# friendlymatthew/heif

Hardware: AMD Instinct MI355X
Metric: Mpixels/s decoded (bit-exact) on 4032x3024 HEIC batch (higher is better)
Workload: dtype u8

## Files before the change

heif_amd/csrc/kernels/intra.hip:

```cpp
#include "kernels.hpp"
#include "intra_rec.hpp"
#include "xform.hpp"
#if defined(HG_HOST_EMU)
#include <cstdio>
#include <cstdlib>
#endif

namespace hg {

namespace {

constexpr int kMaxWaves = 16;
constexpr int kResidentIntraWaves = 4096;
constexpr size_t kIntraLdsBudget = 128 * 1024;

__constant__ int8_t c_angle[35] = {0, 0, 32, 26, 21, 17, 13, 9, 5, 2, 0, -2, -5, -9, -13, -17, -21, -26,
                                   -32, -26, -21, -17, -13, -9, -5, -2, 0, 2, 5, 9, 13, 17, 21, 26, 32};
__constant__ int16_t c_inv_angle[35] = {0, 0, 0, 0, 0, 0, 0, 0, 0, 0, 0, -4096, -1638, -910, -630, -482, -390, -315,
                                        -256, -315, -390, -482, -630, -910, -1638, -4096, 0, 0, 0, 0, 0, 0, 0, 0, 0};

struct alignas(16) IntraScratch {
    int16_t left[66];
    int16_t top[66];
    int16_t fl[66];
// ... 373 lines not shown
            const int p0 = *ang_ref(main_, side, inv, a + idx + 1), p1 = *ang_ref(main_, side, inv, a + idx + 2);
            pv = ((32 - fact) * p0 + fact * p1 + 16) >> 5;
            if (cidx == 0 && n < 32) {
                if (mode == 26) {
                    const int v = min(max(tp[1] + ((lf[1 + y] - lf[0]) >> 1), 0), maxv);
                    pv = x == 0 ? v : pv;
                }
                if (mode == 10) {
                    const int v = min(max(lf[1] + ((tp[1 + x] - tp[0]) >> 1), 0), maxv);
                    pv = y == 0 ? v : pv;
                }
            }
        }
        const int li = ((y0 + y) << w.lsx) + x0 + x;
        if (pcm) pv = 0;
        if (cbf) pv += (n <= 8 && o == lane) ? r0 : rt[y * w.rp + x];
        pv = min(max(pv, 0), maxv);
        w.cur[li] = (Pel)pv;
    };
#if defined(HG_IABL_PRED)
    if (lane == 1000) predict_sample(0);
    if (false)
#elif !defined(HG_HOST_EMU)
    if (n <= 8) {
        if (lane < n * n) predict_sample(lane);
    } else
#endif
    {
        for (int o = lane; o < n * n; o += kWave) predict_sample(o);
    }
    wave_sync();
}

#if !defined(HG_HOST_EMU)
template <typename Pel>
__device__ __attribute__((always_inline)) inline void predict_pair(IntraScratch *L, uint32_t wa, uint32_t wb,
                                                                   const TbWin<Pel> &wc, uint32_t dwin, uint32_t dres,
                                                                   int bd, int lane) {
    static_assert(kWave == 64, "predict_pair splits a 64-lane wave into two halves");
    const int log2n = tba_log2(wa), n = 1 << log2n, mode = tba_mode(wa);
    const int x0 = tba_lx(wa), y0 = tba_ly(wa);
    const int zc = tbb_zc(wb);
    const int h = lane >> 5, sl = lane & 31;
    TbWin<Pel> w = wc;
    const uint32_t dw = h ? dwin : 0u;
    w.cur = wc.cur + dw;
    w.left = wc.left + dw;
    w.above = wc.above + dw;
    const int16_t *rt = wc.rt + (h ? dres : 0u);
    const bool cbf = (wa & (h ? TBA_CBF2 : TBA_CBF)) != 0;
    const bool pcm = (wa & (h ? TBA_PCM2 : TBA_PCM)) != 0;
    const int csl = w.csl;
    const int ns = 4 * n + 1, nch = n == 8 ? 2 : 1;
    int r0 = 0, r1 = 0;
    if (cbf && sl < n * n) r0 = rt[(sl >> log2n) * w.rp + (sl & (n - 1))];
    if (cbf && sl + 32 < n * n) r1 = rt[((sl + 32) >> log2n) * w.rp + ((sl + 32) & (n - 1))];
    int16_t *left = L->left + 33 * h, *top = L->top + 33 * h;
    int val0 = 0, val1 = 0;
    uint32_t hm0 = 0, hm1 = 0;
#pragma unroll
    for (int k = 0; k < 2; ++k) {
        if (k >= nch) break;
        const int s = sl + 32 * k;
        const int xn = s <= 2 * n ? x0 - 1 : x0 + s - 2 * n - 1;
        const int yn = s < 2 * n ? y0 + 2 * n - 1 - s : y0 - 1;
        const bool av = s < ns && xn >= w.minx && yn >= w.miny && xn < w.vw && yn < w.vh &&
                        nb_avail(zc, xn * 2, yn * 2, csl);
        const Pel *srcp = w.at(xn, yn);
        const int vk = av ? (int)*srcp : 0;
        const uint32_t hk = (uint32_t)(__ballot(av) >> (32 * h));
        if (k == 0) {
            val0 = vk;
            hm0 = hk;
        } else {
            val1 = vk;
            hm1 = hk;
        }
    }
    const bool any = (hm0 | hm1) != 0;
#pragma unroll
    for (int k = 0; k < 2; ++k) {
        if (k >= nch) break;
        const int s = sl + 32 * k;
        const uint32_t hmk = k ? hm1 : hm0;
        int sc = k, src = sl;
        if (any && !((hmk >> sl) & 1u)) {
            const uint32_t below = hmk & ((1u << sl) - 1u);
            if (below) {
                src = 31 - __builtin_clz(below);
            } else if (k == 1 && hm0) {
                sc = 0;
                src = 31 - __builtin_clz(hm0);
            } else {
                sc = hm0 ? 0 : 1;
                src = __builtin_ctz(sc ? hm1 : hm0);
            }
        }
        const int v0 = __shfl(val0, 32 * h + src, 64);
        const int v1 = nch > 1 ? __shfl(val1, 32 * h + src, 64) : 0;
        const int v = !any ? (1 << (bd - 1)) : (sc == 0 ? v0 : v1);
        int16_t *dp = s < 2 * n ? left + (2 * n - s) : top + (s - 2 * n);
        if (s < ns) *dp = (int16_t)v;
        if (s == 2 * n) left[0] = (int16_t)v;
    }
    wave_sync();
    const int16_t *lf = left, *tp = top;
    const int maxv = (1 << bd) - 1;
    int dc = 0;
    const int ang = tbb_ang(wb), inv = tbb_inv(wb);
    const int16_t *main_ = mode >= 18 ? tp : lf, *side = mode >= 18 ? lf : tp;
    if (mode == 1) {
        const int sum = group_sum(sl < 2 * n ? (sl < n ? tp[1 + sl] : lf[1 + sl - n]) : 0, 2 * n);
        const int s0 = __builtin_amdgcn_readlane(sum, 0), s1 = __builtin_amdgcn_readlane(sum, 32);
        dc = ((h ? s1 : s0) + n) >> (log2n + 1);
    }
    for (int it = 0; it < nch; ++it) {
        const int o = sl + 32 * it;
        if (o < n * n) {
            const int x = o & (n - 1), y = o >> log2n;
            int pv;
            if (mode == 0) {
                pv = ((n - 1 - x) * lf[1 + y] + (x + 1) * tp[1 + n] + (n - 1 - y) * tp[1 + x] + (y + 1) * lf[1 + n] +
                      n) >> (log2n + 1);
            } else if (mode == 1) {
                pv = dc;
            } else {
                const int a = mode >= 18 ? x : y, b = mode >= 18 ? y : x;
                const int idx = ((b + 1) * ang) >> 5, fact = ((b + 1) * ang) & 31;
                const int p0 = *ang_ref(main_, side, inv, a + idx + 1), p1 = *ang_ref(main_, side, inv, a + idx + 2);
                pv = ((32 - fact) * p0 + fact * p1 + 16) >> 5;
            }
            if (pcm) pv = 0;
            if (cbf) pv += it ? r1 : r0;
            pv = min(max(pv, 0), maxv);
            w.cur[((y0 + y) << w.lsx) + x0 + x] = (Pel)pv;
        }
    }
    wave_sync();
}
#endif

}

#ifndef HG_INTRA_WPE
#define HG_INTRA_WPE 5
#endif
#if HG_INTRA_WPE > 0
#define HG_INTRA_ATTR __attribute__((amdgpu_waves_per_eu(HG_INTRA_WPE)))
#else
#define HG_INTRA_ATTR
#endif
constexpr size_t kXfTablesBytes = sizeof(XfTab);
constexpr size_t kXfDBytes = 32 * kXfDStride32 * sizeof(int16_t), kXfGBytes = 32 * 32 * sizeof(int16_t);
constexpr size_t kXfWaveBytes = kXfDBytes + kXfGBytes + 16;
static_assert(kXfTablesBytes % 16 == 0 && kXfWaveBytes % 16 == 0, "transform scratch alignment");
constexpr int kIntraPlanes = 0, kIntraStream = 1;

#if defined(HG_HOST_EMU)
struct LaneWord {
    uint32_t v[64];
    uint32_t at(int l) const { return v[l]; }
};
struct WalkStats {
    std::atomic<uint64_t> records{0}, ok{0}, pairs{0}, ctus{0}, blocks{0};
    std::atomic<uint64_t> pair_splits{0};
    std::atomic<uint64_t> ctu_lane0{0};
    std::atomic<uint64_t> blocks_no_ctu{0};
    std::atomic<uint64_t> rows_lt64{0}, rows_gt128{0};
    std::atomic<uint64_t> second_rows{0};
    std::atomic<uint64_t> tb32_strong{0}, luma4{0}, pcm{0};
};
static WalkStats g_walk;
static bool walk_stats_on() {
    static const bool on = [] {
        const char *e = std::getenv("HEIFGPU_INTRA_STATS");
        return e && std::atoi(e) != 0;
    }();
    return on;
}
#else
struct LaneWord {
    uint32_t v = 0;
    __device__ __forceinline__ uint32_t at(int l) const { return (uint32_t)__builtin_amdgcn_readlane((int)v, l); }
};
#endif
constexpr uint32_t kGaveUp = ~0u;
constexpr uint64_t kRedoPatience = 200000000ull;

template <typename Pel, int CF, int Mode>
__device__ __attribute__((always_inline)) inline void intra_body(const BatchArgs &a, unsigned char *smem) {
    constexpr bool Poll = Mode == kIntraStream;
    constexpr bool XfInline = Poll;
    const int nw = (int)HG_UNI(blockDim.x >> 6);
    const int pic = a.pic0 + blockIdx.x;
    const int wave = (int)HG_UNI(threadIdx.x >> 6), lane = threadIdx.x & 63;
    const PicDesc pd = a.pics[pic];
    if (pd.flags & PD_ASSEMBLY) return;
    if (Poll && a.stream_redo && hg_load_agent(a.xntu + a.total_rows + pic) != 0) return;
    const SeqParams sp = a.seqs[pd.seq];
    const int W = sp.width, H = sp.height, log2ctb = sp.log2_ctb;
    const int wctb = (W + (1 << log2ctb) - 1) >> log2ctb, hctb = (H + (1 << log2ctb) - 1) >> log2ctb;
    constexpr int chroma = CF;
    const int cw = chroma ? W >> chroma_sx(chroma) : 0, ch = chroma ? H >> chroma_sy(chroma) : 0;
    const int ncomp = chroma ? 3 : 1;
    const bool strong = (sp.flags & SP_STRONG_INTRA) != 0;
    const WinLayout lay = win_layout(log2ctb, chroma, (int)sizeof(Pel));
    uint32_t *progress = reinterpret_cast<uint32_t *>(smem);
    Frame<Pel, CF> F;
    F.blk = smem + 64 + (size_t)wave * lay.bytes;
    F.recon = reinterpret_cast<Pel *>(a.recon + pd.recon_off);
    F.resid = a.resid + pd.resid_off;
    F.init(log2ctb, W, H, cw, ch);
    XfScratch X{};
    if constexpr (XfInline) {
        unsigned char *tab = smem + 64 + (size_t)nw * lay.bytes;
        unsigned char *xw = tab + kXfTablesBytes + (size_t)wave * kXfWaveBytes;
        X = XfScratch{reinterpret_cast<int16_t *>(xw), reinterpret_cast<int16_t *>(xw + kXfDBytes),
                      reinterpret_cast<int32_t *>(xw + kXfDBytes + kXfGBytes), reinterpret_cast<const XfTab *>(tab)};
        xf_tables(reinterpret_cast<XfTab *>(tab), lane);
    }
    IntraScratch *S = reinterpret_cast<IntraScratch *>(F.blk);
    progress[wave] = 0;
    __syncthreads();
    const uint32_t stride = (uint32_t)wctb + 1;
    const bool split = a.intra_split != 0 && ncomp == 3;
    const int cls = split ? (wave & 1) : 0, rw = split ? wave >> 1 : wave, nrw = split ? nw >> 1 : nw;
    const int k0 = split && cls ? 1 : 0, k1 = split && !cls ? 1 : ncomp;
    const int prev_wave = split ? ((rw + nrw - 1) % nrw) * 2 + cls : (wave + nw - 1) % nw;
    const bool wpp = (sp.flags & SP_WPP) != 0;
    bool gave_up = false;
    const TbGeom G{log2ctb, chroma, W, H, cw, ch};
    const WinOffs wo = win_offs(F);
    constexpr int SX = chroma_sx(CF), SY = chroma_sy(CF);
    const uint32_t dwin = F.b1 / (uint32_t)sizeof(Pel);
    const uint32_t dres = (uint32_t)cw * (uint32_t)ch;
#if defined(HG_HOST_EMU)
    const bool stats = walk_stats_on() && cls == 0 && !(Poll && a.stream_redo);
    const bool stats_c = walk_stats_on() && k0 <= 1 && k1 > 1;
#endif
    for (int r = rw; r < hctb; r += nrw) {
        uint32_t ntu = Poll ? 0u : a.row_counts[2 * (pd.row_off + r)];
        bool row_done = !Poll;
        const TuRec *tus = a.tus + pd.tu_off + (uint64_t)r * pd.tu_cap_row;
        const CoefSrc<Poll> coefs{a.coefs + pd.coef_off + (uint64_t)r * pd.coef_cap_row};
        int cur = -1;
        auto finish_ctu = [&]() {
            _Pragma("nounroll") for (int k = 0; k < 3; ++k) {
                if (k >= ncomp) break;
                if (k < k0 || k >= k1) continue;
                const Win<Pel> w = F.win(k, cur, r);
                Pel *const plane = F.plane(k);
                const int PW = F.pw(k), PH = F.ph(k);
                const int vw = min(w.csx, PW - w.cx0), vh = min(w.csy, PH - w.cy0);
                if (vw == w.csx && !(PW & 3) && !(reinterpret_cast<uintptr_t>(plane) & (4 * sizeof(Pel) - 1))) {
                    const int lq = __builtin_ctz((unsigned)w.csx) - 2;
                    for (int o = lane; o < (vh << lq); o += kWave) {
                        const int x = (o & ((1 << lq) - 1)) << 2, y = o >> lq;
                        *reinterpret_cast<Quad<Pel> *>(plane + (size_t)(w.cy0 + y) * PW + w.cx0 + x) =
                            *reinterpret_cast<const Quad<Pel> *>(w.cur + y * w.csx + x);
                    }
                } else {
                    for (int o = lane; o < vw * vh; o += kWave) {
                        const int x = o % vw, y = o / vw;
                        plane[(size_t)(w.cy0 + y) * PW + w.cx0 + x] = w.cur[y * w.csx + x];
                    }
                }
                for (int y = lane; y < w.csy; y += kWave) w.left[y] = w.cur[y * w.csx + w.csx - 1];
            }
            wave_sync();
            HG_FENCE_REL();
            hg_atomic_store(&progress[wave], (uint32_t)r * stride + (uint32_t)cur + 1u);
        };
        auto start_ctu = [&](int c) -> bool {
            if (r > 0) {
                const uint32_t need = (uint32_t)(r - 1) * stride + (uint32_t)min(c + 2, wctb);
                for (uint32_t spin = 0;; ++spin) {
                    const uint32_t v = (uint32_t)HG_UNI(hg_atomic_load(&progress[prev_wave]));
                    if (Poll && v == kGaveUp) return false;
                    if (v >= need) break;
                    if (spin > (1u << 24)) {
                        if (lane == 0) atomicOr(&a.status[pic], ST_SUBSTREAM_END);
                        break;
                    }
                    HG_SLEEP();
                }
                HG_FENCE_ACQ();
            }
            _Pragma("nounroll") for (int k = 0; k < 3; ++k) {
                if (k >= ncomp) break;
                if (k < k0 || k >= k1) continue;
                const Win<Pel> w = F.win(k, c, r);
                const Pel *const plane = F.plane(k);
                const int PW = F.pw(k);
                const int yg = w.cy0 - 1;
                for (int i = lane; i <= 2 * w.csx; i += kWave) {
                    const int xg = w.cx0 - 1 + i;
                    w.above[i] = (yg >= 0 && xg >= 0 && xg < PW) ? plane[(size_t)yg * PW + xg] : (Pel)0;
                }
            }
            wave_sync();
            return true;
        };
#if defined(HG_HOST_EMU)
        if (stats) {
            g_walk.rows_lt64 += ntu < 64 && !Poll;
            g_walk.rows_gt128 += ntu > 128 && !Poll;
            g_walk.second_rows += r != rw;
        }
#endif
        bool stop = false;
        for (uint32_t t = 0; !stop;) {
            if constexpr (Poll) {
                if (t >= ntu && !row_done) {
                    const uint32_t *pw = a.xprog + pd.row_off + (wpp ? r : 0);
                    const uint32_t *nw_ = a.xntu + pd.row_off + r;
                    const uint32_t fin = (uint32_t)(r + 1) * (uint32_t)wctb;
                    const uint64_t patience = (uint64_t)a.stream_patience_us * 100u;
                    uint32_t seen_n = ~0u, seen_p = ~0u;
                    uint64_t t_last = 0;
                    for (;;) {
                        if (!a.stream_redo && !patience) {
                            gave_up = true;
                            break;
                        }
                        const uint32_t n_ = (uint32_t)HG_UNI(hg_load_agent(nw_));
                        if (n_ > t) {
                            ntu = n_;
                            break;
                        }
                        const uint32_t pv = (uint32_t)HG_UNI(hg_load_agent(pw));
                        if (pv >= fin) {
                            ntu = (uint32_t)HG_UNI(hg_load_agent(nw_));
                            row_done = true;
                            break;
                        }
                        const uint64_t now = hg_clock_10ns();
                        if (n_ != seen_n || pv != seen_p) {
                            seen_n = n_;
                            seen_p = pv;
                            t_last = now;
                        } else if (now - t_last > (a.stream_redo ? kRedoPatience : patience)) {
                            if (!a.stream_redo) {
                                gave_up = true;
                            } else {
                                if (lane == 0) atomicOr(&a.status[pic], ST_SUBSTREAM_END);
                                row_done = true;
                            }
                            break;
                        }
                        HG_STREAM_SLEEP();
                    }
                    if (gave_up) break;
                    HG_ACQ_AGENT();
                }
            }
            if (t >= ntu) break;
            const uint32_t base = t & ~63u;
            LaneWord wa, wb, wc, wctu;
#if !defined(HG_HOST_EMU)
            uint4 tblk = make_uint4(0, 0, 0, 0);
#endif
            auto form = [&](int l, uint32_t &A, uint32_t &B, uint32_t &C, uint32_t &ctu) {
                A = B = C = ctu = 0;
                const uint32_t i = base + (uint32_t)l;
                if (i < t || i >= ntu) return;
                TuRec q;
#if defined(HG_HOST_EMU)
                q = tus[i];
#else
                if constexpr (Poll) {
                    const uint64_t *p = reinterpret_cast<const uint64_t *>(tus + i);
// ... 338 lines not shown
```

heif_amd/csrc/kernels/transform.hip:

```cpp
#include "xform.hpp"

namespace hg {

namespace {

#ifndef HG_XF_WAVES
#define HG_XF_WAVES 4
#endif
constexpr int kWaves = HG_XF_WAVES;

#define wave_sync() HG_WAVE_SYNC()

}

#if !defined(HG_XF_WPE)
#define HG_XF_WPE 7
#endif
__global__ void __launch_bounds__(kWaves * 64) __attribute__((amdgpu_waves_per_eu(HG_XF_WPE))) k_transform(BatchArgs a) {
    HG_BLOCK_SHARED __attribute__((aligned(16))) int16_t dtile[kWaves][32 * kXfDStride32];
    HG_BLOCK_SHARED __attribute__((aligned(16))) int16_t gtile[kWaves][32 * 32];
    HG_BLOCK_SHARED int32_t extent[kWaves][2];
    HG_BLOCK_SHARED XfTab s_tab;
#if defined(HG_HOST_EMU)
    xf_tables(&s_tab, 0, 1);
#else
    xf_tables(&s_tab, (int)threadIdx.x, (int)blockDim.x);
#endif
    const int16_t *s_mt = s_tab.mt;
    __syncthreads();
    const int pic = a.pic0 + blockIdx.y, row = blockIdx.x;
    const PicDesc pd = a.pics[pic];
    if (pd.flags & PD_ASSEMBLY) return;
    const SeqParams sp = a.seqs[pd.seq];
    const int hctb = (sp.height + (1 << sp.log2_ctb) - 1) >> sp.log2_ctb;
    if (row >= hctb) return;
    const int wave = (int)HG_UNI(threadIdx.x >> 6), lane = threadIdx.x & 63;
    const uint32_t ntu = a.row_counts[2 * (pd.row_off + row)];
    const TuRec *tus = a.tus + pd.tu_off + (uint64_t)row * pd.tu_cap_row;
    const CoefSrc<false> coefs{a.coefs + pd.coef_off + (uint64_t)row * pd.coef_cap_row};
    const int W = sp.width, H = sp.height;
    const int cw = HG_UNI(sp.chroma_format ? W >> chroma_sx(sp.chroma_format) : 0);
    const int ch = HG_UNI(sp.chroma_format ? H >> chroma_sy(sp.chroma_format) : 0);
    int16_t HG_GAS *const res0 = (int16_t HG_GAS *)(a.resid + pd.resid_off);
    int16_t HG_GAS *res_plane[3] = {res0, res0 + (size_t)W * H, res0 + (size_t)W * H + (size_t)cw * ch};
    const int pitch[3] = {W, cw, cw};
    const bool scaling = (sp.flags & SP_SCALING_LIST) != 0;
    int16_t *d = dtile[wave];
    int16_t *g = gtile[wave];

    {
        const uint32_t mine = ntu > (uint32_t)wave ? (ntu - (uint32_t)wave + kWaves - 1) / kWaves : 0;
        auto want4 = [&](const TuRec &tu) -> bool {
            const int cidx = tu.flags & TU_CIDX_MASK;
            return (tu.flags & TU_CBF) && tu.log2 == 2 && cidx <= 2 && tu.x + 4 <= pitch[cidx] &&
                   tu.y + 4 <= (cidx ? ch : H);
        };
        auto round4 = [&](auto &&grp) {
            for (int vl = lane; vl < 64; vl += kWave) d[vl] = 0;
            wave_sync();
            for (int vl = lane; vl < 64; vl += kWave) {
                TuRec tu;
                const int l16 = vl & 15;
                if (!grp(vl, tu)) continue;
                const int cidx = tu.flags & TU_CIDX_MASK;
                const int bd = cidx ? sp.bit_depth_c : sp.bit_depth_y;
                int pos, dv;
                if (tu.flags & TU_PCM) {
                    if (l16 >= (int)tu.ncoef) continue;
                    const Coef c = coefs.word(tu.coef + (uint32_t)l16);
                    pos = (int)(c & 15u);
                    dv = (int)(int16_t)(c >> 16);
                } else {
                    if (tu.ncoef < 4) continue;
                    const SbRec r = load_rec(coefs, tu.coef);
                    if (!((r.sig() >> l16) & 1u)) continue;
                    const int above = l16 < 15 ? __builtin_popcountll(r.esc() >> (4 * l16 + 4)) : 0;
                    dv = r.level(l16, above, coefs);
                    pos = r.pos(l16, 2);
                }
                if (!(tu.flags & TU_BYPASS)) {
                    const int qp = tu.qp, bd_shift = bd - 3;
                    const int ls = c_level_scale[qp % 6] << (qp / 6);
                    const int m =
                        scaling ? a.sf[sp.sf_off + sf_size_offset(0) + (uint32_t)cidx * 16u + (uint32_t)pos] : 16;
                    dv = clip16(((int64_t)dv * m * ls + ((int64_t)1 << (bd_shift - 1))) >> bd_shift);
                }
                d[(vl & 48) + ((pos & 3) << 2) + (pos >> 2)] = (int16_t)dv;
            }
            wave_sync();
            for (int vl = lane; vl < 64; vl += kWave) {
                TuRec tu;
                if (!grp(vl, tu) || (tu.flags & (TU_BYPASS | TU_TSKIP))) continue;
                const int y = (vl & 15) >> 2, x = vl & 3;
                const uint32_t *pa = reinterpret_cast<const uint32_t *>(mt_of(s_mt, 2, (tu.flags & TU_DST) != 0) + y * 4);
                const uint32_t *pb = reinterpret_cast<const uint32_t *>(d + (vl & 48) + x * 4);
                const int s = dot2_i16(pa[1], pb[1], dot2_i16(pa[0], pb[0], 0));
                g[vl] = (int16_t)min(max((s + 64) >> 7, -32768), 32767);
            }
            wave_sync();
            for (int vl = lane; vl < 64; vl += kWave) {
                TuRec tu;
                if (!grp(vl, tu)) continue;
                const int cidx = tu.flags & TU_CIDX_MASK;
                const int bd2 = 20 - (cidx ? sp.bit_depth_c : sp.bit_depth_y);
                const int y = (vl & 15) >> 2, x = vl & 3;
                const int16_t *dq = d + (vl & 48), *gq = g + (vl & 48);
                int r;
                if (tu.flags & TU_BYPASS) {
                    r = dq[x * 4 + y];
                } else if (tu.flags & TU_TSKIP) {
                    r = (dq[x * 4 + y] * (1 << 7) + (1 << (bd2 - 1))) >> bd2;
                } else {
                    const uint32_t *pa = reinterpret_cast<const uint32_t *>(mt_of(s_mt, 2, (tu.flags & TU_DST) != 0) + x * 4);
                    const uint32_t *pb = reinterpret_cast<const uint32_t *>(gq + y * 4);
                    const int s = dot2_i16(pa[1], pb[1], dot2_i16(pa[0], pb[0], 0));
                    r = (s + (1 << (bd2 - 1))) >> bd2;
                }
                res_plane[cidx][(size_t)(tu.y + y) * pitch[cidx] + tu.x + x] = (int16_t)clip16(r);
            }
            wave_sync();
        };
#if defined(HG_HOST_EMU)
        for (uint32_t j = 0; j < mine; j += 4) {
            round4([&](int vl, TuRec &tu) -> bool {
                const uint32_t jq = j + (uint32_t)(vl >> 4);
                if (jq >= mine) return false;
                tu = tus[(uint32_t)wave + kWaves * jq];
                return want4(tu);
            });
        }
#else
        static_assert(kWave == 64, "one record per lane");
        for (uint32_t c0 = 0; c0 < mine; c0 += 64) {
            const uint32_t jl = c0 + (uint32_t)lane;
            uint4 rec = make_uint4(0, 0, 0, 0);
            if (jl < mine) rec = *reinterpret_cast<const uint4 *>(tus + (uint32_t)wave + kWaves * jl);
            TuRec rl;
            __builtin_memcpy(&rl, &rec, sizeof(rl));
            uint64_t todo = __ballot(jl < mine && want4(rl));
            while (todo) {
                int src = -1;
                for (int q = 0; q < 4 && todo; ++q) {
                    const int jq = __builtin_ctzll(todo);
                    todo &= todo - 1;
                    if (q == (lane >> 4)) src = jq;
                }
                const int sl = src < 0 ? 0 : src;
                const uint4 r = make_uint4((uint32_t)__shfl((int)rec.x, sl, 64), (uint32_t)__shfl((int)rec.y, sl, 64),
                                           (uint32_t)__shfl((int)rec.z, sl, 64), (uint32_t)__shfl((int)rec.w, sl, 64));
                TuRec tu_c;
                __builtin_memcpy(&tu_c, &r, sizeof(tu_c));
                const bool ok_c = src >= 0;
                round4([&](int, TuRec &tu) -> bool {
                    tu = tu_c;
                    return ok_c;
                });
            }
        }
#endif
    }

    auto pass_b = [&](const TuRec &tu) {
        const int cidx = tu.flags & TU_CIDX_MASK;
        transform_tb(tu, coefs, sp, a.sf, XfScratch{d, g, extent[wave], &s_tab},
                     res_plane[cidx] + (size_t)tu.y * pitch[cidx] + tu.x, pitch[cidx], lane);
    };
    auto wanted = [&](const TuRec &tu) {
        const int cidx = tu.flags & TU_CIDX_MASK, n = 1 << tu.log2;
        return (tu.flags & TU_CBF) && tu.log2 != 2 && tu.log2 <= 5 && cidx <= 2 && tu.x + n <= pitch[cidx] &&
               tu.y + n <= (cidx ? ch : H);
    };
#if defined(HG_HOST_EMU)
    for (uint32_t t = wave; t < ntu; t += kWaves)
        if (wanted(tus[t])) pass_b(tus[t]);
#else
    for (uint32_t t0 = wave; t0 < ntu; t0 += 64u * kWaves) {
        const uint32_t t = t0 + (uint32_t)lane * kWaves;
        uint4 rec = make_uint4(0, 0, 0, 0);
        if (t < ntu) rec = *reinterpret_cast<const uint4 *>(tus + t);
        TuRec mine;
        __builtin_memcpy(&mine, &rec, sizeof(mine));
        uint64_t todo = __ballot(t < ntu && wanted(mine));
        while (todo) {
            const int j = __builtin_ctzll(todo);
            todo &= todo - 1;
            const uint4 r = make_uint4((uint32_t)__builtin_amdgcn_readlane((int)rec.x, j),
                                       (uint32_t)__builtin_amdgcn_readlane((int)rec.y, j),
                                       (uint32_t)__builtin_amdgcn_readlane((int)rec.z, j),
                                       (uint32_t)__builtin_amdgcn_readlane((int)rec.w, j));
            TuRec tu;
            __builtin_memcpy(&tu, &r, sizeof(tu));
            pass_b(tu);
        }
    }
#endif
}

__global__ void __launch_bounds__(kWaves * 64) k_paint_flags(BatchArgs a) {
    const int pic = a.pic0 + blockIdx.y, row = blockIdx.x;
    const PicDesc pd = a.pics[pic];
    if (pd.flags & PD_ASSEMBLY) return;
    const SeqParams sp = a.seqs[pd.seq];
    const int hctb = (sp.height + (1 << sp.log2_ctb) - 1) >> sp.log2_ctb;
    if (row >= hctb) return;
    const int w4 = (sp.width + 3) >> 2, h4 = (sp.height + 3) >> 2;
    uint8_t *flg = a.maps + pd.map_off + (size_t)w4 * h4;
    const uint32_t ntu = min(a.row_counts[2 * (pd.row_off + row)], pd.tu_cap_row);
    const TuRec *tus = a.tus + pd.tu_off + (uint64_t)row * pd.tu_cap_row;
    const int wave = (int)(threadIdx.x >> 6), lane = threadIdx.x & 63;
    for (uint32_t t0 = 64u * wave; t0 < ntu; t0 += 64u * kWaves) {
        for (int vl = lane; vl < 64; vl += kWave) {
            const uint32_t t = t0 + (uint32_t)vl;
            if (t >= ntu) continue;
            const TuRec tu = tus[t];
            if ((tu.flags & (TU_CIDX_MASK | TU_PCM)) || tu.log2 < 2 || tu.log2 > 5) continue;
            const int nb = 1 << (tu.log2 - 2), gx0 = tu.x >> 2, gy0 = tu.y >> 2;
            if (gx0 >= w4 || gy0 >= h4) continue;
            const int wx = gx0 + nb <= w4 ? nb : w4 - gx0, hy = gy0 + nb <= h4 ? nb : h4 - gy0;
            const uint8_t nf = (tu.flags & TU_BYPASS) ? MF_NOFILT : 0;
            for (int y = 0; y < hy; ++y) {
                uint8_t *r = flg + (size_t)(gy0 + y) * w4 + gx0;
                const uint8_t h = (uint8_t)((y == 0 ? MF_EDGE_H : 0) | nf);
                const uint64_t v = (0x0101010101010101ull * h) | (uint64_t)MF_EDGE_V;
                if (wx == 8) {
                    __builtin_memcpy(r, &v, 8);
                } else if (wx == 4) {
                    __builtin_memcpy(r, &v, 4);
                } else {
                    for (int x = 0; x < wx; ++x) r[x] = (uint8_t)(v >> (8 * x));
                }
            }
        }
    }
    uint8_t *qmap = a.maps + pd.map_off;
    const int wctb = (sp.width + (1 << sp.log2_ctb) - 1) >> sp.log2_ctb;
    const uint32_t cap = cu_cap_row(wctb, sp.log2_ctb);
    const uint32_t ncu = min(a.cu_counts[pd.row_off + row], cap);
    const uint32_t *cus = a.cus + cu_list_off(pd.sao_off, a.max_log2ctb) + (uint64_t)row * cap;
    for (uint32_t t0 = 64u * wave; t0 < ncu; t0 += 64u * kWaves) {
        for (int vl = lane; vl < 64; vl += kWave) {
            const uint32_t t = t0 + (uint32_t)vl;
            if (t >= ncu) continue;
            const uint32_t w = cus[t];
            const int log2 = (int)((w >> 20) & 15u);
            if (log2 < 3 || log2 > 6) continue;
            const int nb = 1 << (log2 - 2), gx0 = (int)(w & 0xffffu) << 1;
            const int gy0 = (row << (sp.log2_ctb - 2)) + ((int)((w >> 16) & 15u) << 1);
            if (gx0 >= w4 || gy0 >= h4) continue;
            const int wx = gx0 + nb <= w4 ? nb : w4 - gx0, hy = gy0 + nb <= h4 ? nb : h4 - gy0;
            const uint64_t v = 0x0101010101010101ull * (uint64_t)(w >> 24);
            for (int y = 0; y < hy; ++y) {
                uint8_t *r = qmap + (size_t)(gy0 + y) * w4 + gx0;
                int x = 0;
                for (; x + 8 <= wx; x += 8) __builtin_memcpy(r + x, &v, 8);
                if (x + 4 <= wx) {
                    __builtin_memcpy(r + x, &v, 4);
                    x += 4;
                }
                for (; x < wx; ++x) r[x] = (uint8_t)v;
            }
        }
    }
}

#if defined(HG_HOST_EMU)
void emu_transform(const BatchArgs &a) {
    emu_launch(k_transform, a.max_rows, a.n_pics, kWaves, a);
    if (a.flags_from_recs) emu_launch(k_paint_flags, a.max_rows, a.n_pics, kWaves, a);
}
#else
hipError_t launch_transform(const BatchArgs &a, hipStream_t s) {
    hipLaunchKernelGGL(k_transform, dim3(a.max_rows, a.n_pics), dim3(kWaves * 64), 0, s, a);
    if (a.flags_from_recs) hipLaunchKernelGGL(k_paint_flags, dim3(a.max_rows, a.n_pics), dim3(kWaves * 64), 0, s, a);
    return hipGetLastError();
}
#endif

}
```

heif_amd/csrc/kernels/xform.hpp:

```cpp
#pragma once
#include "kernels.hpp"
#include "tables.hpp"

namespace hg {
namespace {

struct TransMatrix {
    int8_t m[32][32];
};
constexpr TransMatrix make_matrix() {
    TransMatrix t{};
    constexpr int odd[16] = {90, 90, 88, 85, 82, 78, 73, 67, 61, 54, 46, 38, 31, 22, 13, 4};
    constexpr int e2[8] = {90, 87, 80, 70, 57, 43, 25, 9};
    constexpr int e4[4] = {89, 75, 50, 18};
    int cv[33] = {};
    cv[0] = 64;
    cv[8] = 83;
    cv[16] = 64;
    cv[24] = 36;
    cv[32] = 0;
    for (int i = 0; i < 16; ++i) cv[2 * i + 1] = odd[i];
    for (int i = 0; i < 8; ++i) cv[2 * (2 * i + 1)] = e2[i];
    for (int i = 0; i < 4; ++i) cv[4 * (2 * i + 1)] = e4[i];
    for (int k = 0; k < 32; ++k)
        for (int n = 0; n < 32; ++n) {
            int j = ((2 * n + 1) * k) % 128;
            int v = j <= 32 ? cv[j] : j <= 64 ? -cv[64 - j] : j <= 96 ? -cv[j - 64] : cv[128 - j];
            t.m[k][n] = (int8_t)v;
        }
    return t;
}
__constant__ TransMatrix c_tm = make_matrix();
__constant__ int8_t c_dst[4][4] = {{29, 55, 74, 84}, {74, 74, 0, -74}, {84, -29, -74, 55}, {55, -84, 74, -29}};
__constant__ int16_t c_level_scale[6] = {40, 45, 51, 57, 64, 72};

#define xf_sync() HG_WAVE_SYNC()

__device__ __forceinline__ int clip16(int64_t v) { return v < -32768 ? -32768 : (v > 32767 ? 32767 : (int)v); }

template <bool Coherent>
struct CoefSrc {
    const Coef *p;
    __device__ __forceinline__ uint32_t word(uint32_t i) const {
#if !defined(HG_HOST_EMU)
        if constexpr (Coherent) return __hip_atomic_load(p + i, __ATOMIC_RELAXED, __HIP_MEMORY_SCOPE_AGENT);
#endif
        return p[i];
    }
};

struct SbRec {
    uint32_t w0, w1, w2, w3;
    __device__ __forceinline__ uint32_t sig() const { return w0 & 0xffffu; }
    __device__ __forceinline__ uint64_t nib() const { return (uint64_t)w1 | ((uint64_t)w2 << 32); }
    __device__ __forceinline__ uint64_t esc() const {
        const uint64_t x = nib();
        return x & (x >> 1) & (x >> 2) & (x >> 3) & 0x1111111111111111ull;
    }
    __device__ __forceinline__ uint32_t esc0() const { return w3 >> 9; }
    __device__ __forceinline__ int pos(int nn, int log2n) const {
        const uint32_t sc = (w3 >> 6) & 3u;
        const uint64_t sw = sc == 0 ? kScan4Pos[0] : (sc == 1 ? kScan4Pos[1] : kScan4Pos[2]);
        const uint32_t pp = (uint32_t)(sw >> (4 * nn)) & 15u;
        const int x = (int)((w3 & 7u) << 2) + (int)(pp & 3u), y = (int)(((w3 >> 3) & 7u) << 2) + (int)(pp >> 2);
        return (y << log2n) + x;
    }
    template <class Src>
    __device__ __forceinline__ int sum_abs(const Src &row) const {
        const uint64_t x = nib();
        const uint64_t t = (x & 0x0f0f0f0f0f0f0f0full) + ((x >> 4) & 0x0f0f0f0f0f0f0f0full);
        int s = __builtin_popcount(sig()) + (int)((t * 0x0101010101010101ull) >> 56);
        const int ne = __builtin_popcountll(esc());
        for (int k = 0; k < ne; ++k) s += (int)row.word(esc0() - (uint32_t)k) - 16;
        return s;
    }
    template <class Src>
    __device__ __forceinline__ int level(int nn, int esc_above, const Src &row) const {
        const int a = (int)((nib() >> (4 * nn)) & 15u);
        const int abs_v = a < 15 ? a + 1 : (int)row.word(esc0() - (uint32_t)esc_above);
        const uint32_t s = sig();
        bool neg;
        if (((w3 >> 8) & 1u) && nn == __builtin_ctz(s)) {
            neg = (sum_abs(row) & 1) != 0;
        } else {
            const int rank = __builtin_popcount(s >> (nn + 1));
            neg = ((w0 << rank) >> 31) != 0;
        }
        const int v = neg ? -abs_v : abs_v;
        return v < -32768 ? -32768 : (v > 32767 ? 32767 : v);
    }
};
template <bool Coherent>
__device__ __forceinline__ SbRec load_rec(const CoefSrc<Coherent> &src, uint32_t i) {
#if defined(HG_HOST_EMU)
    const Coef *p = src.p + i;
    return SbRec{p[0], p[1], p[2], p[3]};
#else
    if constexpr (Coherent) {
        const uint64_t *q = reinterpret_cast<const uint64_t *>(src.p + i);
        const uint64_t lo = __hip_atomic_load(q, __ATOMIC_RELAXED, __HIP_MEMORY_SCOPE_AGENT);
        const uint64_t hi = __hip_atomic_load(q + 1, __ATOMIC_RELAXED, __HIP_MEMORY_SCOPE_AGENT);
        return SbRec{(uint32_t)lo, (uint32_t)(lo >> 32), (uint32_t)hi, (uint32_t)(hi >> 32)};
    }
    const uint4 v = *reinterpret_cast<const uint4 *>(src.p + i);
    return SbRec{v.x, v.y, v.z, v.w};
#endif
}


constexpr int kXfDStride32 = 32 + 2;
constexpr int kMt4Dct = 8 * 10 + 16 * 18 + 32 * 34, kMt4Dst = kMt4Dct + 16;
constexpr int kMtElems = kMt4Dst + 16;
__device__ __forceinline__ int mt_off(int log2n) { return log2n == 3 ? 0 : (log2n == 4 ? 8 * 10 : 8 * 10 + 16 * 18); }

struct alignas(16) XfTab {
    int16_t mt[kMtElems];
};
static_assert(sizeof(XfTab) % 16 == 0 && (sizeof(int16_t) * kMtElems) % 16 == 0, "XfTab layout");

struct XfScratch {
    int16_t *d, *g;
    int32_t *extent;
    const XfTab *tab;
};

constexpr XfTab make_xf_tab() {
    XfTab t{};
    const TransMatrix m = make_matrix();
    constexpr int dst4[4][4] = {{29, 55, 74, 84}, {74, 74, 0, -74}, {84, -29, -74, 55}, {55, -84, 74, -29}};
    for (int i = 0; i < kMtElems; ++i) {
        if (i >= kMt4Dct) {
            const int k = i & 3, y = (i >> 2) & 3;
            t.mt[i] = (int16_t)(i >= kMt4Dst ? dst4[k][y] : m.m[k * 8][y]);
            continue;
        }
        const int l2 = i < 80 ? 3 : (i < 80 + 288 ? 4 : 5), n = 1 << l2, sn = n + 2;
        const int k = i - (l2 == 3 ? 0 : (l2 == 4 ? 80 : 80 + 288));
        const int y = k / sn, j = k % sn;
        t.mt[i] = (int16_t)(j < n ? m.m[j << (5 - l2)][y] : 0);
    }
    return t;
}
__constant__ XfTab c_xf = make_xf_tab();

__device__ __forceinline__ void xf_tables(XfTab *dst, int tid, int nth = kWave) {
    for (int i = tid; i < (int)(sizeof(XfTab) / 4); i += nth)
        reinterpret_cast<uint32_t *>(dst)[i] = reinterpret_cast<const uint32_t *>(&c_xf)[i];
}

#if !defined(HG_HOST_EMU) && !defined(HG_XF_NO_MFMA)
typedef int xf_v4i __attribute__((ext_vector_type(4)));
typedef int xf_v16i __attribute__((ext_vector_type(16)));
__device__ __forceinline__ int xf_hi(uint32_t w0, uint32_t w1) {
    return (int)__builtin_amdgcn_perm(w1, w0, 0x07050301u);
}
__device__ __forceinline__ int xf_lo(uint32_t w0, uint32_t w1) {
    return (int)(__builtin_amdgcn_perm(w1, w0, 0x06040200u) ^ 0x80808080u);
}
__device__ __forceinline__ int xf_hi4(int g0, int g1, int g2, int g3) {
    return (int)(__builtin_amdgcn_perm((uint32_t)g1, (uint32_t)g0, 0x0c0c0501u) |
                 (__builtin_amdgcn_perm((uint32_t)g3, (uint32_t)g2, 0x0c0c0501u) << 16));
}
__device__ __forceinline__ int xf_lo4(int g0, int g1, int g2, int g3) {
    return (int)((__builtin_amdgcn_perm((uint32_t)g1, (uint32_t)g0, 0x0c0c0400u) |
                  (__builtin_amdgcn_perm((uint32_t)g3, (uint32_t)g2, 0x0c0c0400u) << 16)) ^ 0x80808080u);
}
__device__ __forceinline__ int xf_b8(uint32_t w0, uint32_t w1) {
    return (int)__builtin_amdgcn_perm(w1, w0, 0x06040200u);
}
template <class DstPtr>
__device__ __forceinline__ void transform_mfma(const int16_t *dT, int sn, int log2n, const int16_t *mt, DstPtr dst,
                                               int pitch, int bd2, int lane) {
    const int n = 1 << log2n, r = lane & 31, h = lane >> 5;
    const bool live = r < n, live1 = live && 16 * h < n;
    const uint32_t *pm = reinterpret_cast<const uint32_t *>(mt + (live ? r : 0) * sn);
    const uint32_t *pm1 = pm + (live1 ? 8 * h : 0);
    const xf_v4i b1 = {live1 ? xf_b8(pm1[0], pm1[1]) : 0, live1 ? xf_b8(pm1[2], pm1[3]) : 0,
                       live1 ? xf_b8(pm1[4], pm1[5]) : 0, live1 ? xf_b8(pm1[6], pm1[7]) : 0};
    const uint32_t *pm2 = pm + 2 * h;
    const bool live2 = live && n == 32;
    const xf_v4i b2 = {live ? xf_b8(pm2[0], pm2[1]) : 0, live ? xf_b8(pm2[4], pm2[5]) : 0,
                       live2 ? xf_b8(pm2[8], pm2[9]) : 0, live2 ? xf_b8(pm2[12], pm2[13]) : 0};
    int cs = __builtin_amdgcn_sdot4(b1.x, 0x01010101, 0, false);
    cs = __builtin_amdgcn_sdot4(b1.y, 0x01010101, cs, false);
    cs = __builtin_amdgcn_sdot4(b1.z, 0x01010101, cs, false);
    cs = __builtin_amdgcn_sdot4(b1.w, 0x01010101, cs, false);
    const int corr = 128 * (cs + __shfl_xor(cs, 32, 64));
    const uint32_t *pa = reinterpret_cast<const uint32_t *>(dT + r * sn + 16 * h);
    const xf_v4i ah = {xf_hi(pa[0], pa[1]), xf_hi(pa[2], pa[3]), xf_hi(pa[4], pa[5]), xf_hi(pa[6], pa[7])};
    const xf_v4i al = {xf_lo(pa[0], pa[1]), xf_lo(pa[2], pa[3]), xf_lo(pa[4], pa[5]), xf_lo(pa[6], pa[7])};
    xf_v16i acc = {};
    acc = __builtin_amdgcn_mfma_i32_32x32x32_i8(ah, b1, acc, 0, 0, 0);
#pragma unroll
    for (int i = 0; i < 16; ++i) acc[i] = (acc[i] << 8) + corr;
    acc = __builtin_amdgcn_mfma_i32_32x32x32_i8(al, b1, acc, 0, 0, 0);
    int g[16];
#pragma unroll
    for (int i = 0; i < 16; ++i) g[i] = min(max((acc[i] + 64) >> 7, -32768), 32767);
    const xf_v4i gh = {xf_hi4(g[0], g[1], g[2], g[3]), xf_hi4(g[4], g[5], g[6], g[7]),
                       xf_hi4(g[8], g[9], g[10], g[11]), xf_hi4(g[12], g[13], g[14], g[15])};
    const xf_v4i gl = {xf_lo4(g[0], g[1], g[2], g[3]), xf_lo4(g[4], g[5], g[6], g[7]),
                       xf_lo4(g[8], g[9], g[10], g[11]), xf_lo4(g[12], g[13], g[14], g[15])};
    acc = xf_v16i{};
    acc = __builtin_amdgcn_mfma_i32_32x32x32_i8(gh, b2, acc, 0, 0, 0);
    const int rnd = 1 << (bd2 - 1);
#pragma unroll
    for (int i = 0; i < 16; ++i) acc[i] = (acc[i] << 8) + corr + rnd;
    acc = __builtin_amdgcn_mfma_i32_32x32x32_i8(gl, b2, acc, 0, 0, 0);
    auto out = [&](int i) {
        const int y = (i & 3) + 8 * (i >> 2) + 4 * h;
        dst[y * pitch + r] = (int16_t)min(max(acc[i] >> bd2, -32768), 32767);
    };
    if (n == 32) {
#pragma unroll
        for (int i = 0; i < 16; ++i) out(i);
    } else if (r < n) {
#pragma unroll
        for (int i = 0; i < 8; ++i) out(i);
    }
}
#endif

__device__ __forceinline__ const int16_t *mt_of(const int16_t *mt, int log2n, bool dst_tr) {
    return log2n == 2 ? mt + (dst_tr ? kMt4Dst : kMt4Dct) : mt + mt_off(log2n);
}
__device__ __forceinline__ int mt_stride(int log2n) { return log2n == 2 ? 4 : (1 << log2n) + 2; }

__device__ __forceinline__ int dot2_i16(uint32_t a, uint32_t b, int s) {
#if defined(HG_HOST_EMU)
    return s + (int)(int16_t)(a & 0xffffu) * (int)(int16_t)(b & 0xffffu) + (int)(int16_t)(a >> 16) * (int)(int16_t)(b >> 16);
#else
    typedef short short2_t __attribute__((ext_vector_type(2)));
    short2_t va, vb;
    __builtin_memcpy(&va, &a, 4);
    __builtin_memcpy(&vb, &b, 4);
    return __builtin_amdgcn_sdot2(va, vb, s, false);
#endif
}

template <bool Coherent, class DstPtr>
__device__ __forceinline__ void transform_tb(const TuRec &tu, const CoefSrc<Coherent> &coefs, const SeqParams &sp,
                                             const uint8_t *sf, const XfScratch &X, DstPtr dst, int pitch, int lane) {
    int16_t *d = X.d, *g = X.g;
    const bool scaling = (sp.flags & SP_SCALING_LIST) != 0;
    const int cidx = tu.flags & TU_CIDX_MASK;
    const int log2n = tu.log2, n = 1 << log2n;
    if (log2n < 2 || log2n > 5 || cidx > 2) return;
    const int bd = cidx ? sp.bit_depth_c : sp.bit_depth_y;
    const bool bypass = (tu.flags & TU_BYPASS) != 0, ts = (tu.flags & TU_TSKIP) != 0;
    const bool dots = !bypass && !ts;
    const int sn = mt_stride(log2n);
    for (int i = lane; i < (dots ? n * sn : n * n) / 2; i += kWave) reinterpret_cast<int32_t *>(d)[i] = 0;
    if (lane == 0) X.extent[0] = X.extent[1] = 0;
    xf_sync();
    const int qp = tu.qp;
    const int bd_shift = bd + log2n - 5;
    const int64_t rnd = (int64_t)1 << (bd_shift - 1);
    const int ls = c_level_scale[qp % 6] << (qp / 6);
    const bool use_m = scaling && !(ts && n > 4);
    const uint8_t *mtab = sf + sp.sf_off + sf_size_offset(log2n - 2) + (uint32_t)cidx * (uint32_t)(n * n);
    int my_row = 0, my_col = 0;
    auto put = [&](int pos, int v) {
        pos &= n * n - 1;
        int dv;
        if (bypass) {
            dv = v;
        } else {
            const int m = use_m ? mtab[pos] : 16;
            dv = clip16(((int64_t)v * m * ls + rnd) >> bd_shift);
        }
        d[dots ? (pos & (n - 1)) * sn + (pos >> log2n) : pos] = (int16_t)dv;
        my_row = max(my_row, pos >> log2n);
        my_col = max(my_col, pos & (n - 1));
    };
    if (tu.flags & TU_PCM) {
        for (int k = lane; k < tu.ncoef; k += kWave) {
            const Coef c = coefs.word(tu.coef + (uint32_t)k);
            put((int)(c & 0xffffu), (int)(int16_t)(c >> 16));
        }
    } else {
        const int nrec = (int)(tu.ncoef >> 2);
        for (int q = lane; q < 16 * nrec; q += kWave) {
            const SbRec r = load_rec(coefs, tu.coef + 4u * (uint32_t)(q >> 4));
            const int nn = q & 15;
            if (!((r.sig() >> nn) & 1u)) continue;
            const int above = nn < 15 ? __builtin_popcountll(r.esc() >> (4 * nn + 4)) : 0;
            put(r.pos(nn, log2n), r.level(nn, above, coefs));
        }
    }
    if (my_row) atomicMax(&X.extent[0], my_row);
    if (my_col) atomicMax(&X.extent[1], my_col);
    xf_sync();
    const int rows = X.extent[0] + 1, cols = X.extent[1] + 1;
    const int bd2 = 20 - bd;
    if (bypass || ts) {
        const int ts_shift = 5 + log2n;
        for (int i = lane; i < n * n; i += kWave) {
            int r = d[i];
            if (!bypass) r = (r * (1 << ts_shift) + (1 << (bd2 - 1))) >> bd2;
            dst[(i >> log2n) * pitch + (i & (n - 1))] = (int16_t)clip16(r);
        }
        xf_sync();
        return;
    }
    const bool dst_tr = (tu.flags & TU_DST) != 0;
    if (!dst_tr && rows == 1 && cols == 1) {
        const int g0 = clip16(((int64_t)64 * d[0] + 64) >> 7);
        const int16_t r = (int16_t)clip16(((int64_t)64 * g0 + (1 << (bd2 - 1))) >> bd2);
        for (int i = lane; i < n * n; i += kWave) dst[(i >> log2n) * pitch + (i & (n - 1))] = r;
        xf_sync();
        return;
    }
#if !defined(HG_HOST_EMU) && !defined(HG_XF_NO_MFMA)
    if (log2n >= 4) {
        transform_mfma(d, sn, log2n, mt_of(X.tab->mt, log2n, false), dst, pitch, bd2, lane);
        xf_sync();
        return;
    }
#endif
    const int16_t *mt = mt_of(X.tab->mt, log2n, dst_tr);
    const int rows4 = (rows + 3) & ~3, cols4 = (cols + 3) & ~3;
    const int lc = cols4 > 4 ? 32 - __builtin_clz((unsigned)(cols4 - 1)) : 2;
    for (int o = lane; o < (n << lc); o += kWave) {
        const int y = o >> lc, x = o & ((1 << lc) - 1);
        if (x >= cols4) continue;
        const uint32_t *pa = reinterpret_cast<const uint32_t *>(mt + y * sn);
        const uint32_t *pb = reinterpret_cast<const uint32_t *>(d + x * sn);
        int s = 0;
#pragma unroll 2
        for (int j = 0; j < rows4 / 2; j += 2) {
            s = dot2_i16(pa[j], pb[j], s);
            s = dot2_i16(pa[j + 1], pb[j + 1], s);
        }
        g[y * n + x] = (int16_t)min(max((s + 64) >> 7, -32768), 32767);
    }
    xf_sync();
    for (int o = lane; o < n * n; o += kWave) {
        const int y = o >> log2n, x = o & (n - 1);
        const uint32_t *pa = reinterpret_cast<const uint32_t *>(mt + x * sn);
        const uint32_t *pb = reinterpret_cast<const uint32_t *>(g + y * n);
        int s = 0;
#pragma unroll 2
        for (int j = 0; j < cols4 / 2; j += 2) {
            s = dot2_i16(pa[j], pb[j], s);
            s = dot2_i16(pa[j + 1], pb[j + 1], s);
        }
        dst[y * pitch + x] = (int16_t)min(max((s + (1 << (bd2 - 1))) >> bd2, -32768), 32767);
    }
    xf_sync();
}

}
}
```

Measured before the change: 28710.

## Add DC-only fast path and ballot-based extents to transform, drop LDS extent atomics

Adds an early path in transform_tb for TUs whose single coefficient record holds only a DC value. It skips zeroing the scratch tile and the dequant pass, and writes the constant residual with 16-byte vector stores when alignment allows. It replaces the per-wave LDS extent array and its atomicMax reductions with subblock-position maxima computed from the records and reduced across the wave with ballots. It also software-pipelines the record loads and swaps the constant-memory level-scale lookup for a packed-immediate computation. The new code adds debug ablation macros and relies on the subblock-position extents matching what the old coefficient-position extents produced.

Result: faster. 30040, median of 6 (+4.6%).

```diff
diff --git a/heif_amd/csrc/kernels/intra.hip b/heif_amd/csrc/kernels/intra.hip
--- a/heif_amd/csrc/kernels/intra.hip
+++ b/heif_amd/csrc/kernels/intra.hip
@@ -549,7 +549,7 @@
 #endif
 constexpr size_t kXfTablesBytes = sizeof(XfTab);
 constexpr size_t kXfDBytes = 32 * kXfDStride32 * sizeof(int16_t), kXfGBytes = 32 * 32 * sizeof(int16_t);
-constexpr size_t kXfWaveBytes = kXfDBytes + kXfGBytes + 16;
+constexpr size_t kXfWaveBytes = kXfDBytes + kXfGBytes;
 static_assert(kXfTablesBytes % 16 == 0 && kXfWaveBytes % 16 == 0, "transform scratch alignment");
 constexpr int kIntraPlanes = 0, kIntraStream = 1;
 
@@ -613,7 +613,7 @@
         unsigned char *tab = smem + 64 + (size_t)nw * lay.bytes;
         unsigned char *xw = tab + kXfTablesBytes + (size_t)wave * kXfWaveBytes;
         X = XfScratch{reinterpret_cast<int16_t *>(xw), reinterpret_cast<int16_t *>(xw + kXfDBytes),
-                      reinterpret_cast<int32_t *>(xw + kXfDBytes + kXfGBytes), reinterpret_cast<const XfTab *>(tab)};
+                      reinterpret_cast<const XfTab *>(tab)};
         xf_tables(reinterpret_cast<XfTab *>(tab), lane);
     }
     IntraScratch *S = reinterpret_cast<IntraScratch *>(F.blk);
diff --git a/heif_amd/csrc/kernels/transform.hip b/heif_amd/csrc/kernels/transform.hip
--- a/heif_amd/csrc/kernels/transform.hip
+++ b/heif_amd/csrc/kernels/transform.hip
@@ -19,7 +19,6 @@
 __global__ void __launch_bounds__(kWaves * 64) __attribute__((amdgpu_waves_per_eu(HG_XF_WPE))) k_transform(BatchArgs a) {
     HG_BLOCK_SHARED __attribute__((aligned(16))) int16_t dtile[kWaves][32 * kXfDStride32];
     HG_BLOCK_SHARED __attribute__((aligned(16))) int16_t gtile[kWaves][32 * 32];
-    HG_BLOCK_SHARED int32_t extent[kWaves][2];
     HG_BLOCK_SHARED XfTab s_tab;
 #if defined(HG_HOST_EMU)
     xf_tables(&s_tab, 0, 1);
@@ -48,6 +47,7 @@
     int16_t *d = dtile[wave];
     int16_t *g = gtile[wave];
 
+#if !defined(HG_XABL_PASS_A)
     {
         const uint32_t mine = ntu > (uint32_t)wave ? (ntu - (uint32_t)wave + kWaves - 1) / kWaves : 0;
         auto want4 = [&](const TuRec &tu) -> bool {
@@ -79,11 +79,10 @@
                     pos = r.pos(l16, 2);
                 }
                 if (!(tu.flags & TU_BYPASS)) {
-                    const int qp = tu.qp, bd_shift = bd - 3;
-                    const int ls = c_level_scale[qp % 6] << (qp / 6);
+                    const int bd_shift = bd - 3, ls = xf_level_scale(tu.qp);
                     const int m =
                         scaling ? a.sf[sp.sf_off + sf_size_offset(0) + (uint32_t)cidx * 16u + (uint32_t)pos] : 16;
-                    dv = clip16(((int64_t)dv * m * ls + ((int64_t)1 << (bd_shift - 1))) >> bd_shift);
+                    dv = xf_scale64(dv, m, ls, bd_shift);
                 }
                 d[(vl & 48) + ((pos & 3) << 2) + (pos >> 2)] = (int16_t)dv;
             }
@@ -159,10 +158,15 @@
         }
 #endif
     }
+#endif
 
     auto pass_b = [&](const TuRec &tu) {
+#if defined(HG_XABL_TB) && !defined(HG_HOST_EMU)
+        asm volatile("" ::"s"(tu.coef), "s"((uint32_t)tu.ncoef), "s"((uint32_t)tu.x), "s"((uint32_t)tu.qp));
+        return;
+#endif
         const int cidx = tu.flags & TU_CIDX_MASK;
-        transform_tb(tu, coefs, sp, a.sf, XfScratch{d, g, extent[wave], &s_tab},
+        transform_tb(tu, coefs, sp, a.sf, XfScratch{d, g, &s_tab},
                      res_plane[cidx] + (size_t)tu.y * pitch[cidx] + tu.x, pitch[cidx], lane);
     };
     auto wanted = [&](const TuRec &tu) {
diff --git a/heif_amd/csrc/kernels/xform.hpp b/heif_amd/csrc/kernels/xform.hpp
--- a/heif_amd/csrc/kernels/xform.hpp
+++ b/heif_amd/csrc/kernels/xform.hpp
@@ -1,6 +1,7 @@
 #pragma once
 #include "kernels.hpp"
 #include "tables.hpp"
+#include "xform_rec.hpp"
 
 namespace hg {
 namespace {
@@ -32,7 +33,6 @@
 }
 __constant__ TransMatrix c_tm = make_matrix();
 __constant__ int8_t c_dst[4][4] = {{29, 55, 74, 84}, {74, 74, 0, -74}, {84, -29, -74, 55}, {55, -84, 74, -29}};
-__constant__ int16_t c_level_scale[6] = {40, 45, 51, 57, 64, 72};
 
 #define xf_sync() HG_WAVE_SYNC()
 
@@ -120,7 +120,6 @@
 
 struct XfScratch {
     int16_t *d, *g;
-    int32_t *extent;
     const XfTab *tab;
 };
 
@@ -238,6 +237,40 @@
 #endif
 }
 
+struct alignas(16) XfRow8 {
+    uint32_t w[4];
+};
+#if defined(__HIP_DEVICE_COMPILE__)
+__device__ __forceinline__ void xf_store8(int16_t HG_GAS *p, const XfRow8 &v) {
+    *reinterpret_cast<XfRow8 HG_GAS *>(p) = v;
+}
+#endif
+__device__ __forceinline__ void xf_store8(int16_t *p, const XfRow8 &v) { *reinterpret_cast<XfRow8 *>(p) = v; }
+
+__device__ __forceinline__ int xf_wave_max(int v, int bits) {
+#if defined(HG_HOST_EMU)
+    (void)bits;
+    return v;
+#else
+    uint64_t alive = ~0ull;
+    int m = 0;
+    for (int b = bits - 1; b >= 0; --b) {
+        const uint64_t t = __ballot((v >> b) & 1) & alive;
+        if (t) {
+            m |= 1 << b;
+            alive = t;
+        }
+    }
+    return m;
+#endif
+}
+
+#if !defined(HG_HOST_EMU) && !defined(HG_XF_NO_MFMA)
+constexpr bool kXfMfma = true;
+#else
+constexpr bool kXfMfma = false;
+#endif
+
 template <bool Coherent, class DstPtr>
 __device__ __forceinline__ void transform_tb(const TuRec &tu, const CoefSrc<Coherent> &coefs, const SeqParams &sp,
                                              const uint8_t *sf, const XfScratch &X, DstPtr dst, int pitch, int lane) {
@@ -248,51 +281,71 @@
     if (log2n < 2 || log2n > 5 || cidx > 2) return;
     const int bd = cidx ? sp.bit_depth_c : sp.bit_depth_y;
     const bool bypass = (tu.flags & TU_BYPASS) != 0, ts = (tu.flags & TU_TSKIP) != 0;
+    const bool pcm = (tu.flags & TU_PCM) != 0, dst_tr = (tu.flags & TU_DST) != 0;
     const bool dots = !bypass && !ts;
     const int sn = mt_stride(log2n);
+    const int bd_shift = bd + log2n - 5, bd2 = 20 - bd;
+    const int ls = xf_level_scale(tu.qp);
+    const bool use_m = scaling && !(ts && n > 4);
+    const int nrec = pcm ? 0 : (int)(tu.ncoef >> 2);
+    SbRec r0{0, 0, 0, 0};
+    if (nrec > 0) r0 = load_rec(coefs, tu.coef + 4u * (uint32_t)min(lane >> 4, nrec - 1));
+    if (nrec == 1 && dots && !dst_tr && !use_m && HG_UNI((int)xf_dc_record(r0.w0, r0.w3))) {
+        const int v = r0.level(0, 0, coefs);
+        const int dv = xf_scale64(v, 16, ls, bd_shift);
+        const int g0 = xf_clip16((64 * dv + 64) >> 7);
+        const int16_t r = (int16_t)xf_clip16((64 * g0 + (1 << (bd2 - 1))) >> bd2);
+        if (log2n >= 3 && (((uintptr_t)dst | (uintptr_t)(2 * pitch)) & 15u) == 0) {
+            const uint32_t rr = (uint32_t)(uint16_t)r * 0x10001u;
+            const XfRow8 row{{rr, rr, rr, rr}};
+            for (int i = lane; i < (n * n) >> 3; i += kWave)
+                xf_store8(dst + (i >> (log2n - 3)) * pitch + ((i & ((n >> 3) - 1)) << 3), row);
+        } else {
+            for (int i = lane; i < n * n; i += kWave) dst[(i >> log2n) * pitch + (i & (n - 1))] = r;
+        }
+        xf_sync();
+        return;
+    }
     for (int i = lane; i < (dots ? n * sn : n * n) / 2; i += kWave) reinterpret_cast<int32_t *>(d)[i] = 0;
-    if (lane == 0) X.extent[0] = X.extent[1] = 0;
     xf_sync();
-    const int qp = tu.qp;
-    const int bd_shift = bd + log2n - 5;
-    const int64_t rnd = (int64_t)1 << (bd_shift - 1);
-    const int ls = c_level_scale[qp % 6] << (qp / 6);
-    const bool use_m = scaling && !(ts && n > 4);
     const uint8_t *mtab = sf + sp.sf_off + sf_size_offset(log2n - 2) + (uint32_t)cidx * (uint32_t)(n * n);
-    int my_row = 0, my_col = 0;
     auto put = [&](int pos, int v) {
         pos &= n * n - 1;
         int dv;
         if (bypass) {
             dv = v;
         } else {
-            const int m = use_m ? mtab[pos] : 16;
-            dv = clip16(((int64_t)v * m * ls + rnd) >> bd_shift);
+            dv = xf_scale64(v, use_m ? mtab[pos] : 16, ls, bd_shift);
         }
         d[dots ? (pos & (n - 1)) * sn + (pos >> log2n) : pos] = (int16_t)dv;
-        my_row = max(my_row, pos >> log2n);
-        my_col = max(my_col, pos & (n - 1));
     };
-    if (tu.flags & TU_PCM) {
+    const bool ext = dots && (!kXfMfma || log2n < 4);
+    int xs_max = 0, ys_max = 0;
+    if (pcm) {
         for (int k = lane; k < tu.ncoef; k += kWave) {
             const Coef c = coefs.word(tu.coef + (uint32_t)k);
             put((int)(c & 0xffffu), (int)(int16_t)(c >> 16));
         }
     } else {
-        const int nrec = (int)(tu.ncoef >> 2);
-        for (int q = lane; q < 16 * nrec; q += kWave) {
-            const SbRec r = load_rec(coefs, tu.coef + 4u * (uint32_t)(q >> 4));
+        SbRec r = r0;
+        for (int q = lane; q < 16 * nrec;) {
             const int nn = q & 15;
-            if (!((r.sig() >> nn) & 1u)) continue;
-            const int above = nn < 15 ? __builtin_popcountll(r.esc() >> (4 * nn + 4)) : 0;
-            put(r.pos(nn, log2n), r.level(nn, above, coefs));
-        }
-    }
-    if (my_row) atomicMax(&X.extent[0], my_row);
-    if (my_col) atomicMax(&X.extent[1], my_col);
+            if (ext) {
+                xs_max = max(xs_max, (int)(r.w3 & 7u));
+                ys_max = max(ys_max, (int)((r.w3 >> 3) & 7u));
+            }
+            if ((r.sig() >> nn) & 1u) {
+                const int above = nn < 15 ? __builtin_popcountll(r.esc() >> (4 * nn + 4)) : 0;
+                put(r.pos(nn, log2n), r.level(nn, above, coefs));
+            }
+            q += kWave;
+            if (q < 16 * nrec) r = load_rec(coefs, tu.coef + 4u * (uint32_t)(q >> 4));
+        }
+    }
     xf_sync();
-    const int rows = X.extent[0] + 1, cols = X.extent[1] + 1;
-    const int bd2 = 20 - bd;
+#if defined(HG_XABL_STAGES)
+    return;
+#endif
     if (bypass || ts) {
         const int ts_shift = 5 + log2n;
         for (int i = lane; i < n * n; i += kWave) {
@@ -303,14 +356,6 @@
         xf_sync();
         return;
     }
-    const bool dst_tr = (tu.flags & TU_DST) != 0;
-    if (!dst_tr && rows == 1 && cols == 1) {
-        const int g0 = clip16(((int64_t)64 * d[0] + 64) >> 7);
-        const int16_t r = (int16_t)clip16(((int64_t)64 * g0 + (1 << (bd2 - 1))) >> bd2);
-        for (int i = lane; i < n * n; i += kWave) dst[(i >> log2n) * pitch + (i & (n - 1))] = r;
-        xf_sync();
-        return;
-    }
 #if !defined(HG_HOST_EMU) && !defined(HG_XF_NO_MFMA)
     if (log2n >= 4) {
         transform_mfma(d, sn, log2n, mt_of(X.tab->mt, log2n, false), dst, pitch, bd2, lane);
@@ -319,7 +364,8 @@
     }
 #endif
     const int16_t *mt = mt_of(X.tab->mt, log2n, dst_tr);
-    const int rows4 = (rows + 3) & ~3, cols4 = (cols + 3) & ~3;
+    int rows4, cols4;
+    xf_extents(xf_wave_max(xs_max, 3), xf_wave_max(ys_max, 3), n, &rows4, &cols4);
     const int lc = cols4 > 4 ? 32 - __builtin_clz((unsigned)(cols4 - 1)) : 2;
     for (int o = lane; o < (n << lc); o += kWave) {
         const int y = o >> lc, x = o & ((1 << lc) - 1);
diff --git a/heif_amd/csrc/kernels/xform_rec.hpp b/heif_amd/csrc/kernels/xform_rec.hpp
--- /dev/null
+++ b/heif_amd/csrc/kernels/xform_rec.hpp
@@ -0,0 +1,37 @@
+#pragma once
+#include <stdint.h>
+
+#include "../common/desc.hpp"
+
+#if !defined(HG_REC_FN)
+#if defined(__HIPCC__) && !defined(HG_HOST_EMU)
+#define HG_REC_FN __host__ __device__ __forceinline__
+#else
+#define HG_REC_FN inline
+#endif
+#endif
+
+namespace hg {
+
+HG_REC_FN int xf_level_scale(int qp) {
+    const uint64_t tab = 40ull | (45ull << 8) | (51ull << 16) | (57ull << 24) | (64ull << 32) | (72ull << 40);
+    const int per = (qp & 255) / 6, rem = (qp & 255) - 6 * per;
+    return (int)((tab >> (8 * rem)) & 0xffu) << (per < 16 ? per : 16);
+}
+
+HG_REC_FN int xf_clip16(int v) { return v < -32768 ? -32768 : (v > 32767 ? 32767 : v); }
+
+HG_REC_FN int xf_scale64(int v, int m, int ls, int bd_shift) {
+    const int64_t t = ((int64_t)v * m * ls + ((int64_t)1 << (bd_shift - 1))) >> bd_shift;
+    return t < -32768 ? -32768 : (t > 32767 ? 32767 : (int)t);
+}
+
+HG_REC_FN bool xf_dc_record(uint32_t w0, uint32_t w3) { return (w0 & 0xffffu) == 1u && (w3 & 63u) == 0u; }
+
+HG_REC_FN void xf_extents(int xs_max, int ys_max, int n, int *rows4, int *cols4) {
+    const bool in = 4 * xs_max < n && 4 * ys_max < n;
+    *rows4 = in ? 4 * (ys_max + 1) : n;
+    *cols4 = in ? 4 * (xs_max + 1) : n;
+}
+
+}
```
